# jianzhangcs/DAGL

Measured on AMD Instinct MI355X. Metric: graph-attn fwd query-patches/s @256x256x64 k=8, higher is better.
Workload: dtype f32

## Files before the change

dagl_amd/csrc/aggregate.hip:

```cpp
#include "dagl_common.h"
#include "aggregate_direct.h"
#include "topk_merge.h"

namespace dagl {


__global__ __launch_bounds__(256) void edge_softmax_fast_kernel(EdgeArgs a) {
    const int lane = threadIdx.x & 63;
    const size_t ql = (size_t)blockIdx.x * 4 + (threadIdx.x >> 6);
    if (ql >= (size_t)a.B * a.L) return;
    int n = a.cnt[ql];
    if (n > DAGL_FAST_CAP) n = DAGL_FAST_CAP;
    int key = 0x7fffffff; float s = 0.f;
    if (lane < n) { key = a.list_idx[ql * DAGL_FAST_CAP + lane]; s = a.list_val[ql * DAGL_FAST_CAP + lane]; }
#pragma unroll
    for (int k2 = 2; k2 <= 64; k2 <<= 1) {
#pragma unroll
        for (int j = k2 >> 1; j > 0; j >>= 1) {
            const int okey = __shfl_xor(key, j);
            const float os = __shfl_xor(s, j);
            const bool up = ((lane & k2) == 0);
            const bool lower = ((lane & j) == 0);
            const bool take = (lower == up) ? (okey < key) : (okey > key);
            if (take) { key = okey; s = os; }
        }
    }
    const float mtq = a.mt[ql], bsq = a.bs[ql];
    const bool valid = lane < n;
    const float lg = valid ? edge_logit(s, mtq, bsq, true) : 0.f;
    double M = wave_max_f64(valid ? (double)lg : -1e300);
    if (n < a.N) M = fmax(M, 0.0);
    const double e = valid ? exp((double)lg - M) : 0.0;
    const double sum = wave_sum_f64(e) + (double)(a.N - n) * exp(-M);
    if (valid) {
        a.nb_idx[ql * a.width + lane] = key;
        a.nb_wgt[ql * a.width + lane] = (float)(e / sum);
        if (a.nb_s != nullptr) a.nb_s[ql * a.width + lane] = s;
    }
    if (lane == 0) a.nb_cnt[ql] = n;
}

__global__ __launch_bounds__(256) void edge_softmax_csr_kernel(EdgeArgs a) {
    const int lane = threadIdx.x & 63;
    const size_t ql = (size_t)blockIdx.x * 4 + (threadIdx.x >> 6);
    if (ql >= (size_t)a.B * a.L) return;
    const int64_t o0 = a.row_off[ql], o1 = a.row_off[ql + 1];
    const int n = (int)(o1 - o0);
    const float mtq = a.mt[ql], bsq = a.bs[ql];
    double M = -1e300;
    for (int64_t o = o0 + lane; o < o1; o += 64) M = fmax(M, (double)edge_logit(a.list_val[o], mtq, bsq, true));
    M = wave_max_f64(M);
    if (n < a.N) M = fmax(M, 0.0);
    double sum = 0.0;
    for (int64_t o = o0 + lane; o < o1; o += 64) sum += exp((double)edge_logit(a.list_val[o], mtq, bsq, true) - M);
    sum = wave_sum_f64(sum) + (double)(a.N - n) * exp(-M);
    for (int64_t o = o0 + lane; o < o1; o += 64) {
        a.nb_idx[o] = a.list_idx[o];
        a.nb_wgt[o] = (float)(exp((double)edge_logit(a.list_val[o], mtq, bsq, true) - M) / sum);
    }
    if (lane == 0) a.nb_cnt[ql] = n;
}

__global__ __launch_bounds__(256) void edge_softmax_topk_kernel(EdgeArgs a, int kslots, unsigned n_blocks) {
    __shared__ float cv[4][TOPK_MAX_CAND];
    __shared__ int ci[4][TOPK_MAX_CAND];
    if (a.run_flags == nullptr) { edge_softmax_topk_unit(a, kslots, cv, ci, blockIdx.x); return; }
    if (a.run_count != nullptr && *a.run_count == 0) return;
    const int nqg = (a.L + 127) / 128;
    for (size_t blk = blockIdx.x; blk < n_blocks; blk += gridDim.x) {
        const size_t q0 = blk * 4, q1 = (q0 + 3 < (size_t)a.B * a.L - 1) ? q0 + 3 : (size_t)a.B * a.L - 1;
        const size_t b0 = q0 / a.L, b1 = q1 / a.L;
        if (a.run_flags[b0 * nqg + (q0 - b0 * a.L) / 128] == 0 && a.run_flags[b1 * nqg + (q1 - b1 * a.L) / 128] == 0) continue;
        edge_softmax_topk_unit(a, kslots, cv, ci, blk);
    }
}

__global__ void row_stats_kernel(size_t n_rows, const float* __restrict__ nb_wgt, const int32_t* __restrict__ nb_cnt,
                                 const int64_t* __restrict__ row_off, int width, int32_t* __restrict__ deg,
                                 float* __restrict__ rowsum) {
    const size_t r = (size_t)blockIdx.x * blockDim.x + threadIdx.x;
    if (r >= n_rows) return;
    const int n = nb_cnt[r];
    if (n < 0) return;
    const float* w = nb_wgt + (row_off ? (size_t)row_off[r] : r * width);
    double s = 0.0;
    for (int j = 0; j < n; ++j) s += (double)w[j];
    if (deg) deg[r] = n;
    if (rowsum) rowsum[r] = (float)s;
}

int launch_row_stats(hipStream_t s, size_t n_rows, const float* nb_wgt, const int32_t* nb_cnt, const int64_t* row_off,
                     int width, int32_t* deg, float* rowsum) {
    hipLaunchKernelGGL(row_stats_kernel, dim3((unsigned)((n_rows + 255) / 256)), dim3(256), 0, s, n_rows, nb_wgt,
                       nb_cnt, row_off, width, deg, rowsum);
    DAGL_LAUNCH_CHECK("row_stats_kernel");
    return DAGL_OK;
}

int launch_edge_softmax(hipStream_t s, const EdgeArgs& a) {
    const size_t nq = (size_t)a.B * a.L;
    dim3 grid((unsigned)((nq + 3) / 4)), block(256);
    if (a.mode == DAGL_MODE_ADAPTIVE) {
        if (a.row_off == nullptr) hipLaunchKernelGGL(edge_softmax_fast_kernel, grid, block, 0, s, a);
        else hipLaunchKernelGGL(edge_softmax_csr_kernel, grid, block, 0, s, a);
    } else {
        const int ks = topk_slots(a.k);
        if (a.splits * 2 * ks > TOPK_MAX_CAND) {
            set_error("edge softmax: %d candidates per query exceed %d", a.splits * 2 * ks, TOPK_MAX_CAND);
            return DAGL_ERR_INVALID;
        }
        dim3 g2 = grid;
        if (a.run_flags != nullptr && g2.x > 128) g2.x = 128;
        hipLaunchKernelGGL(edge_softmax_topk_kernel, g2, block, 0, s, a, ks, grid.x);
    }
    DAGL_LAUNCH_CHECK("edge_softmax_kernel");
    return DAGL_OK;
}

__global__ __launch_bounds__(256) void aggregate_direct_kernel(AggArgs a) {
    __shared__ int sh_of[AGG_STAGE];
    __shared__ float sh_w[AGG_STAGE];
    aggregate_direct_block(a, blockIdx.y, blockIdx.x, sh_of, sh_w);
}

int launch_aggregate_direct(hipStream_t s, const AggArgs& a) {
    dim3 grid((unsigned)a.g.L, a.B), block(256);
    hipLaunchKernelGGL(aggregate_direct_kernel, grid, block, 0, s, a);
    DAGL_LAUNCH_CHECK("aggregate_direct_kernel");
    return DAGL_OK;
}

template <int KU>
__global__ __launch_bounds__(256) void gather_rows_kernel(int L, int k, int P4, const int32_t* __restrict__ idx,
                                                          const float* __restrict__ wgt,
                                                          const float4* __restrict__ values,
                                                          float4* __restrict__ out) {
    const size_t t = (size_t)blockIdx.x * blockDim.x + threadIdx.x;
    if (t >= (size_t)L * P4) return;
    const int q = (int)(t / P4), r = (int)(t % P4);
    const int32_t* ip = idx + (size_t)q * k;
    const float* wp = wgt + (size_t)q * k;
    float4 acc = make_float4(0.f, 0.f, 0.f, 0.f);
    int j = 0;
    for (; j + KU <= k; j += KU) {
        int id[KU]; float w[KU]; float4 v[KU];
#pragma unroll
        for (int u = 0; u < KU; ++u) { id[u] = ip[j + u]; w[u] = wp[j + u]; }
#pragma unroll
        for (int u = 0; u < KU; ++u) {
            const bool ok = id[u] >= 0;
            v[u] = values[(size_t)(ok ? id[u] : 0) * P4 + r];
            if (!ok) w[u] = 0.f;
        }
#pragma unroll
        for (int u = 0; u < KU; ++u) {
            acc.x = fmaf(w[u], v[u].x, acc.x); acc.y = fmaf(w[u], v[u].y, acc.y);
            acc.z = fmaf(w[u], v[u].z, acc.z); acc.w = fmaf(w[u], v[u].w, acc.w);
        }
    }
    for (; j < k; ++j) {
        const int id = ip[j];
        if (id < 0) continue;
        const float w = wp[j];
        const float4 v = values[(size_t)id * P4 + r];
        acc.x = fmaf(w, v.x, acc.x); acc.y = fmaf(w, v.y, acc.y);
        acc.z = fmaf(w, v.z, acc.z); acc.w = fmaf(w, v.w, acc.w);
    }
    out[t] = acc;
}

int launch_gather_fixed(hipStream_t s, int L, int k, int P_, const int32_t* idx, const float* wgt,
                        const float* values, float* out) {
    const int P4 = P_ / 4;
    const size_t items = (size_t)L * P4;
    dim3 grid((unsigned)((items + 255) / 256)), block(256);
    if (k % 8 == 0)
        hipLaunchKernelGGL(gather_rows_kernel<8>, grid, block, 0, s, L, k, P4, idx, wgt,
                           reinterpret_cast<const float4*>(values), reinterpret_cast<float4*>(out));
    else
        hipLaunchKernelGGL(gather_rows_kernel<4>, grid, block, 0, s, L, k, P4, idx, wgt,
                           reinterpret_cast<const float4*>(values), reinterpret_cast<float4*>(out));
    DAGL_LAUNCH_CHECK("gather_rows_kernel");
    return DAGL_OK;
}

__global__ __launch_bounds__(256) void fold_kernel(Grid g, const float* __restrict__ agg, float* __restrict__ out,
                                                   int imgs, int heads, RangeTag range) {
    const int b = blockIdx.z;
    const int y = blockIdx.y;
    const int x = blockIdx.x * blockDim.x + threadIdx.x;
    const bool poisoned = (range.word != nullptr && *range.word == range.tag) || (range.veto != nullptr && *range.veto == range.tag);
    if (range.done != nullptr && b == 0 && y == 0 && blockIdx.x == 0 && threadIdx.x == 0) *range.done = range.tag;
    if (x >= g.W) return;
    int r0 = (y - 3 + QS - 1) / QS; if (y - 3 < 0) r0 = 0;
    int r1 = (y + 3) / QS; if (r1 > g.Lh - 1) r1 = g.Lh - 1;
    int c0 = (x - 3 + QS - 1) / QS; if (x - 3 < 0) c0 = 0;
    int c1 = (x + 3) / QS; if (c1 > g.Lw - 1) c1 = g.Lw - 1;
    float4 acc[CH / 4];
#pragma unroll
    for (int u = 0; u < CH / 4; ++u) acc[u] = make_float4(0.f, 0.f, 0.f, 0.f);
    for (int r = r0; r <= r1; ++r) {
        const int kh = y - (QS * r - 3);
        for (int c = c0; c <= c1; ++c) {
            const int kw = x - (QS * c - 3);
            const float4* p = reinterpret_cast<const float4*>(
                agg + ((size_t)b * g.L + (size_t)r * g.Lw + c) * P + (kh * KS + kw) * CH);
#pragma unroll
            for (int u = 0; u < CH / 4; ++u) {
                const float4 v = p[u];
                acc[u].x += v.x; acc[u].y += v.y; acc[u].z += v.z; acc[u].w += v.w;
            }
        }
    }
    float cnt = (float)((r1 - r0 + 1) * (c1 - c0 + 1));
    if (poisoned) cnt = __builtin_nanf("");
    const int head = b / imgs, img = b - head * imgs;
    float* o = out + ((size_t)img * heads + head) * CH * g.N + (size_t)y * g.W + x;
#pragma unroll
    for (int u = 0; u < CH / 4; ++u) {
        o[(size_t)(4 * u + 0) * g.N] = acc[u].x / cnt;
        o[(size_t)(4 * u + 1) * g.N] = acc[u].y / cnt;
        o[(size_t)(4 * u + 2) * g.N] = acc[u].z / cnt;
        o[(size_t)(4 * u + 3) * g.N] = acc[u].w / cnt;
    }
}

__device__ __forceinline__ void key_row_col(int id, int W, float inv_w, int& jy, int& jx) {
    jy = (int)((float)id * inv_w);
    jx = id - jy * W;
    if (jx < 0) { --jy; jx += W; } else if (jx >= W) { ++jy; jx -= W; }
}

__global__ __launch_bounds__(256) void aggregate_fold_kernel(AggArgs a, float* __restrict__ out, int imgs, int heads,
                                                             RangeTag range) {
    const Grid& g = a.g;
    const int b = blockIdx.z;
    const int t = blockIdx.x * blockDim.x + threadIdx.x;
    const int pix = t >> 2, u = t & 3;
    bool poisoned = range.word != nullptr && *range.word == range.tag;
    if (range.done != nullptr && b == 0 && blockIdx.x == 0 && threadIdx.x == 0) *range.done = range.tag;
    if (a.unserved != nullptr && *a.unserved != 0) {
        poisoned = true;
        if (b == 0 && blockIdx.x == 0 && threadIdx.x == 0) *a.unserved_sticky = 1;
    }
    if (pix >= g.N) return;
    const int y = pix / g.W, x = pix - y * g.W;
    int r0 = (y - 3 + QS - 1) / QS; if (y - 3 < 0) r0 = 0;
    int r1 = (y + 3) / QS; if (r1 > g.Lh - 1) r1 = g.Lh - 1;
    int c0 = (x - 3 + QS - 1) / QS; if (x - 3 < 0) c0 = 0;
    int c1 = (x + 3) / QS; if (c1 > g.Lw - 1) c1 = g.Lw - 1;
    const float4* vm = reinterpret_cast<const float4*>(a.b2p + (size_t)b * g.Hp * g.Wp * CH) + u;
    const int W = g.W, Wp = g.Wp;
    const float inv_w = 1.0f / (float)W;
    float4 acc = make_float4(0.f, 0.f, 0.f, 0.f);
    for (int r = r0; r <= r1; ++r) {
        const int kh = y - (QS * r - 3);
        for (int c = c0; c <= c1; ++c) {
            const int kw = x - (QS * c - 3);
            const size_t ql = (size_t)b * g.L + (size_t)r * g.Lw + c;
            const int n = a.nb_cnt[ql];
            const int32_t* ip = a.nb_idx + ql * a.width;
            const float* wp = a.nb_wgt + ql * a.width;
            float4 q = make_float4(0.f, 0.f, 0.f, 0.f);
            int j = 0;
            for (; j + 4 <= n; j += 4) {
                int id[4]; float w[4]; float4 v[4];
#pragma unroll
                for (int e = 0; e < 4; ++e) { id[e] = ip[j + e]; w[e] = wp[j + e]; }
#pragma unroll
                for (int e = 0; e < 4; ++e) {
                    int jy, jx; key_row_col(id[e], W, inv_w, jy, jx);
                    v[e] = vm[((jy + kh) * Wp + jx + kw) * (CH / 4)];
                }
#pragma unroll
                for (int e = 0; e < 4; ++e) {
                    q.x = fmaf(w[e], v[e].x, q.x); q.y = fmaf(w[e], v[e].y, q.y);
                    q.z = fmaf(w[e], v[e].z, q.z); q.w = fmaf(w[e], v[e].w, q.w);
                }
            }
            for (; j < n; ++j) {
                const int id = ip[j]; const float w = wp[j];
                int jy, jx; key_row_col(id, W, inv_w, jy, jx);
                const float4 v = vm[((jy + kh) * Wp + jx + kw) * (CH / 4)];
                q.x = fmaf(w, v.x, q.x); q.y = fmaf(w, v.y, q.y);
                q.z = fmaf(w, v.z, q.z); q.w = fmaf(w, v.w, q.w);
            }
            acc.x += q.x; acc.y += q.y; acc.z += q.z; acc.w += q.w;
        }
    }
    float cnt = (float)((r1 - r0 + 1) * (c1 - c0 + 1));
    if (poisoned) cnt = __builtin_nanf("");
    const int head = b / imgs, img = b - head * imgs;
    float* o = out + ((size_t)img * heads + head) * CH * g.N + (size_t)y * g.W + x;
    o[(size_t)(4 * u + 0) * g.N] = acc.x / cnt;
    o[(size_t)(4 * u + 1) * g.N] = acc.y / cnt;
    o[(size_t)(4 * u + 2) * g.N] = acc.z / cnt;
    o[(size_t)(4 * u + 3) * g.N] = acc.w / cnt;
}

int launch_aggregate_fold(hipStream_t s, const AggArgs& a, float* out, int heads, RangeTag range) {
    dim3 grid((unsigned)(((size_t)a.g.N * 4 + 255) / 256), 1, a.B), block(256);
    hipLaunchKernelGGL(aggregate_fold_kernel, grid, block, 0, s, a, out, a.B / heads, heads, range);
    DAGL_LAUNCH_CHECK("aggregate_fold_kernel");
    return DAGL_OK;
}

int launch_fold(hipStream_t s, int B, const Grid& g, const float* agg, float* out, int heads, RangeTag range) {
    dim3 grid((g.W + 63) / 64, g.H, B), block(64);
    hipLaunchKernelGGL(fold_kernel, grid, block, 0, s, g, agg, out, B / heads, heads, range);
    DAGL_LAUNCH_CHECK("fold_kernel");
    return DAGL_OK;
}

constexpr int MIX_TILES = 4;
__global__ __launch_bounds__(256) void stage_mix_kernel(int HW, const float* __restrict__ cat, const float* __restrict__ x,
                                                        const float* __restrict__ mix_w, const float* __restrict__ mix_b,
                                                        float* __restrict__ out) {
    const int lane = threadIdx.x & 63, wave = threadIdx.x >> 6;
    const int i = lane & 15, g = lane >> 4;
    const int b = blockIdx.y;
    const int pw = (blockIdx.x * 4 + wave) * (16 * MIX_TILES);
    if (pw >= HW) return;
    float w[4][16];
#pragma unroll
    for (int n = 0; n < 4; ++n)
#pragma unroll
        for (int T = 0; T < 16; ++T) w[n][T] = mix_w[(n * 16 + i) * 64 + 4 * T + g];
    float bo[4][4];
#pragma unroll
    for (int n = 0; n < 4; ++n)
#pragma unroll
        for (int r = 0; r < 4; ++r) bo[n][r] = mix_b[n * 16 + 4 * g + r];
    float av[MIX_TILES][16];
#pragma unroll
    for (int t = 0; t < MIX_TILES; ++t) {
        int px = pw + 16 * t + i; if (px >= HW) px = HW - 1;
        const float* cb = cat + (size_t)b * 64 * HW + px;
#pragma unroll
        for (int T = 0; T < 16; ++T) av[t][T] = cb[(size_t)(4 * T + g) * HW];
    }
#pragma unroll
    for (int t = 0; t < MIX_TILES; ++t) {
        f32x4 acc[4];
#pragma unroll
        for (int n = 0; n < 4; ++n) acc[n] = (f32x4){0.f, 0.f, 0.f, 0.f};
#pragma unroll
        for (int T = 0; T < 16; ++T)
#pragma unroll
            for (int n = 0; n < 4; ++n) acc[n] = __builtin_amdgcn_mfma_f32_16x16x4f32(w[n][T], av[t][T], acc[n], 0, 0, 0);
        const int pp = pw + 16 * t + i;
#pragma unroll
        for (int n = 0; n < 4; ++n) {
#pragma unroll
            for (int r = 0; r < 4; ++r) {
                const int o = n * 16 + 4 * g + r;
                if (pp < HW) {
                    const size_t idx = ((size_t)b * 64 + o) * HW + pp;
                    out[idx] = (acc[n][r] + bo[n][r]) + x[idx];
                }
            }
        }
    }
}

int launch_stage_mix(hipStream_t s, int B, int HW, const float* cat, const float* x, const float* mix_w,
                     const float* mix_b, float* out) {
    dim3 grid((HW + 64 * MIX_TILES - 1) / (64 * MIX_TILES), B), block(256);
    hipLaunchKernelGGL(stage_mix_kernel, grid, block, 0, s, HW, cat, x, mix_w, mix_b, out);
    DAGL_LAUNCH_CHECK("stage_mix_kernel");
    return DAGL_OK;
}

}
```

Before: 18.46 million.

## Stage neighbor index/weight lists in per-wave LDS for fold aggregation

Rewrites the aggregate-fold kernel so each wave covers a 16-pixel row segment. The wave cooperatively loads each overlapping query patch's neighbor indices and weights once, precomputes the row/column offsets, and stages them as packed (offset, weight) pairs in LDS in chunks of 8. Each thread then gathers values from LDS instead of re-reading and re-decoding the same neighbor lists from global memory. This removes redundant global loads and integer divides, at the cost of wave-level barriers, more LDS use, and a fallback to the old per-thread path at edges.

```diff
diff --git a/dagl_amd/csrc/aggregate.hip b/dagl_amd/csrc/aggregate.hip
--- a/dagl_amd/csrc/aggregate.hip
+++ b/dagl_amd/csrc/aggregate.hip
@@ -231,19 +231,9 @@
     if (jx < 0) { --jy; jx += W; } else if (jx >= W) { ++jy; jx -= W; }
 }
 
-__global__ __launch_bounds__(256) void aggregate_fold_kernel(AggArgs a, float* __restrict__ out, int imgs, int heads,
-                                                             RangeTag range) {
+__device__ __forceinline__ void aggregate_fold_thread(const AggArgs& a, float* __restrict__ out, int imgs, int heads, int b,
+                                                      int pix, int u, bool poisoned) {
     const Grid& g = a.g;
-    const int b = blockIdx.z;
-    const int t = blockIdx.x * blockDim.x + threadIdx.x;
-    const int pix = t >> 2, u = t & 3;
-    bool poisoned = range.word != nullptr && *range.word == range.tag;
-    if (range.done != nullptr && b == 0 && blockIdx.x == 0 && threadIdx.x == 0) *range.done = range.tag;
-    if (a.unserved != nullptr && *a.unserved != 0) {
-        poisoned = true;
-        if (b == 0 && blockIdx.x == 0 && threadIdx.x == 0) *a.unserved_sticky = 1;
-    }
-    if (pix >= g.N) return;
     const int y = pix / g.W, x = pix - y * g.W;
     int r0 = (y - 3 + QS - 1) / QS; if (y - 3 < 0) r0 = 0;
     int r1 = (y + 3) / QS; if (r1 > g.Lh - 1) r1 = g.Lh - 1;
@@ -298,6 +288,160 @@
     o[(size_t)(4 * u + 3) * g.N] = acc.w / cnt;
 }
 
+constexpr int GF_COLS = 6, GF_SLOTS = 2 * GF_COLS, GF_CHUNK = 8;
+
+__device__ __forceinline__ void gather_fold_window(const int4* pairs, int nrem, const float4* vm, int d, float4& q) {
+    if (nrem == GF_CHUNK) {
+        int4 p[GF_CHUNK / 2]; float4 v[GF_CHUNK];
+#pragma unroll
+        for (int e = 0; e < GF_CHUNK / 2; ++e) p[e] = pairs[e];
+#pragma unroll
+        for (int e = 0; e < GF_CHUNK; ++e) v[e] = vm[(((e & 1) ? p[e >> 1].z : p[e >> 1].x) + d) * (CH / 4)];
+#pragma unroll
+        for (int e = 0; e < GF_CHUNK; ++e) {
+            const float w = __int_as_float((e & 1) ? p[e >> 1].w : p[e >> 1].y);
+            q.x = fmaf(w, v[e].x, q.x); q.y = fmaf(w, v[e].y, q.y);
+            q.z = fmaf(w, v[e].z, q.z); q.w = fmaf(w, v[e].w, q.w);
+        }
+        return;
+    }
+    const int2* pr = reinterpret_cast<const int2*>(pairs);
+    int j = 0;
+    if (nrem >= 4) {
+        int2 p[4]; float4 v[4];
+#pragma unroll
+        for (int e = 0; e < 4; ++e) p[e] = pr[e];
+#pragma unroll
+        for (int e = 0; e < 4; ++e) v[e] = vm[(p[e].x + d) * (CH / 4)];
+#pragma unroll
+        for (int e = 0; e < 4; ++e) {
+            const float w = __int_as_float(p[e].y);
+            q.x = fmaf(w, v[e].x, q.x); q.y = fmaf(w, v[e].y, q.y);
+            q.z = fmaf(w, v[e].z, q.z); q.w = fmaf(w, v[e].w, q.w);
+        }
+        j = 4;
+    }
+    for (; j < nrem; ++j) {
+        const int2 p = pr[j];
+        const float w = __int_as_float(p.y);
+        const float4 v = vm[(p.x + d) * (CH / 4)];
+        q.x = fmaf(w, v.x, q.x); q.y = fmaf(w, v.y, q.y);
+        q.z = fmaf(w, v.z, q.z); q.w = fmaf(w, v.w, q.w);
+    }
+}
+
+__device__ __forceinline__ void wave_lds_order() {
+    __builtin_amdgcn_fence(__ATOMIC_RELEASE, "wavefront");
+    __builtin_amdgcn_wave_barrier();
+    __builtin_amdgcn_fence(__ATOMIC_ACQUIRE, "wavefront");
+}
+
+__global__ __launch_bounds__(256) void aggregate_fold_kernel(AggArgs a, float* __restrict__ out, int imgs, int heads,
+                                                             RangeTag range) {
+    __shared__ int4 slab[4][GF_SLOTS * GF_CHUNK / 2];
+    __shared__ int slab_n[4][GF_SLOTS];
+    const Grid& g = a.g;
+    const int b = blockIdx.z;
+    const int t = blockIdx.x * blockDim.x + threadIdx.x;
+    const int pix = t >> 2, u = t & 3;
+    bool poisoned = range.word != nullptr && *range.word == range.tag;
+    if (range.done != nullptr && b == 0 && blockIdx.x == 0 && threadIdx.x == 0) *range.done = range.tag;
+    if (a.unserved != nullptr && *a.unserved != 0) {
+        poisoned = true;
+        if (b == 0 && blockIdx.x == 0 && threadIdx.x == 0) *a.unserved_sticky = 1;
+    }
+    const int W = g.W, Wp = g.Wp;
+    const int wave = __builtin_amdgcn_readfirstlane(threadIdx.x >> 6), lane = threadIdx.x & 63;
+    const int pix0 = blockIdx.x * 64 + wave * 16;
+    const int y = pix0 / W, x0 = pix0 - y * W;
+    if (pix0 + 15 >= g.N || x0 + 15 >= W) {
+        if (pix < g.N) aggregate_fold_thread(a, out, imgs, heads, b, pix, u, poisoned);
+        return;
+    }
+    const int x = x0 + (lane >> 2);
+    int r0 = (y - 3 + QS - 1) / QS; if (y - 3 < 0) r0 = 0;
+    int r1 = (y + 3) / QS; if (r1 > g.Lh - 1) r1 = g.Lh - 1;
+    int c0 = (x - 3 + QS - 1) / QS; if (x - 3 < 0) c0 = 0;
+    int c1 = (x + 3) / QS; if (c1 > g.Lw - 1) c1 = g.Lw - 1;
+    int C0 = (x0 - 3 + QS - 1) / QS; if (x0 - 3 < 0) C0 = 0;
+    int C1 = (x0 + 15 + 3) / QS; if (C1 > g.Lw - 1) C1 = g.Lw - 1;
+    const int nR = r1 - r0 + 1, nC = C1 - C0 + 1;
+
+    int4* const wslab = slab[wave];
+    int2* const wpair = reinterpret_cast<int2*>(wslab);
+    const float inv_w = 1.0f / (float)W;
+    const int32_t* ip[2]; const float* wp[2]; int nq[2]; bool on[2];
+    const int jl = (lane & 7) < a.width ? (lane & 7) : 0;
+#pragma unroll
+    for (int h = 0; h < 2; ++h) {
+        const int s = (lane + 64 * h) >> 3;
+        const int ri = s >= GF_COLS ? 1 : 0, ci = s - GF_COLS * ri;
+        on[h] = s < GF_SLOTS && ri < nR && ci < nC;
+        const size_t ql = (size_t)b * g.L + (size_t)(r0 + (on[h] ? ri : 0)) * g.Lw + (C0 + (on[h] ? ci : 0));
+        ip[h] = a.nb_idx + ql * a.width; wp[h] = a.nb_wgt + ql * a.width;
+        nq[h] = a.nb_cnt[ql];
+    }
+    int id0[2]; float w0[2];
+#pragma unroll
+    for (int h = 0; h < 2; ++h) { id0[h] = ip[h][jl]; w0[h] = wp[h][jl]; }
+#pragma unroll
+    for (int h = 0; h < 2; ++h) {
+        if (!on[h]) nq[h] = 0;
+        if (on[h] && (lane & 7) == 0) slab_n[wave][(lane + 64 * h) >> 3] = nq[h];
+    }
+    wave_lds_order();
+    const float4* vm = reinterpret_cast<const float4*>(a.b2p + (size_t)b * g.Hp * g.Wp * CH) + u;
+    int nw[2][2];
+    float4 q[2][2];
+#pragma unroll
+    for (int ri = 0; ri < 2; ++ri)
+#pragma unroll
+        for (int ci = 0; ci < 2; ++ci) {
+            q[ri][ci] = make_float4(0.f, 0.f, 0.f, 0.f);
+            nw[ri][ci] = (ri < nR && c0 + ci <= c1) ? slab_n[wave][ri * GF_COLS + (c0 - C0) + ci] : 0;
+        }
+    for (int base = 0;; base += GF_CHUNK) {
+        if (base != 0) {
+            const int j = base + (lane & 7), jc = j < a.width ? j : 0;
+#pragma unroll
+            for (int h = 0; h < 2; ++h) { id0[h] = ip[h][jc]; w0[h] = wp[h][jc]; }
+        }
+#pragma unroll
+        for (int h = 0; h < 2; ++h) {
+            int jy, jx; key_row_col(id0[h], W, inv_w, jy, jx);
+            if (on[h]) wpair[lane + 64 * h] = make_int2(jy * Wp + jx, __float_as_int(w0[h]));
+        }
+        wave_lds_order();
+#pragma unroll
+        for (int ri = 0; ri < 2; ++ri) {
+            const int kh = y - (QS * (r0 + ri) - 3);
+#pragma unroll
+            for (int ci = 0; ci < 2; ++ci) {
+                int nrem = nw[ri][ci] - base; if (nrem > GF_CHUNK) nrem = GF_CHUNK;
+                if (nrem <= 0) continue;
+                const int kw = x - (QS * (c0 + ci) - 3);
+                gather_fold_window(wslab + (ri * GF_COLS + (c0 - C0) + ci) * (GF_CHUNK / 2), nrem, vm, kh * Wp + kw, q[ri][ci]);
+            }
+        }
+        if (!__any(nq[0] > base + GF_CHUNK || nq[1] > base + GF_CHUNK)) break;
+        wave_lds_order();
+    }
+    float4 acc = make_float4(0.f, 0.f, 0.f, 0.f);
+#pragma unroll
+    for (int ri = 0; ri < 2; ++ri)
+#pragma unroll
+        for (int ci = 0; ci < 2; ++ci)
+            if (ri < nR && c0 + ci <= c1) { acc.x += q[ri][ci].x; acc.y += q[ri][ci].y; acc.z += q[ri][ci].z; acc.w += q[ri][ci].w; }
+    float cnt = (float)((r1 - r0 + 1) * (c1 - c0 + 1));
+    if (poisoned) cnt = __builtin_nanf("");
+    const int head = b / imgs, img = b - head * imgs;
+    float* o = out + ((size_t)img * heads + head) * CH * g.N + (size_t)y * g.W + x;
+    o[(size_t)(4 * u + 0) * g.N] = acc.x / cnt;
+    o[(size_t)(4 * u + 1) * g.N] = acc.y / cnt;
+    o[(size_t)(4 * u + 2) * g.N] = acc.z / cnt;
+    o[(size_t)(4 * u + 3) * g.N] = acc.w / cnt;
+}
+
 int launch_aggregate_fold(hipStream_t s, const AggArgs& a, float* out, int heads, RangeTag range) {
     dim3 grid((unsigned)(((size_t)a.g.N * 4 + 255) / 256), 1, a.B), block(256);
     hipLaunchKernelGGL(aggregate_fold_kernel, grid, block, 0, s, a, out, a.B / heads, heads, range);
```

New measurement: 18.40 million. Within noise of the previous version (-0.4%).
